# PacificBiosciences/ccs

Measured on AMD Instinct MI355X. Metric: ZMWs/sec (HiFi reads/sec), 10-pass x 10 kb synthetic, higher is better.
Workload: dtype f32

## Files before the change

ccs_amd/csrc/ccsx_api.cpp:

```cpp
#include <hip/hip_runtime.h>

#include <algorithm>
#include <cmath>
#include <cstdio>
#include <cstdlib>
#include <cstring>
#include <initializer_list>
#include <mutex>
#include <string>
#include <vector>

#include "ccsx.h"
#include "ccsx_internal.h"
#include "ccsx_kernels.h"

#define HIPTRY(expr)                                                                                           \
    do {                                                                                                       \
        hipError_t e_ = (expr);                                                                                \
        if (e_ != hipSuccess) {                                                                                \
            ccsx_set_error(std::string(#expr) + ": " + hipGetErrorString(e_));                                 \
            return -2;                                                                                         \
        }                                                                                                      \
    } while (0)

// ... 330 lines not shown
    for (int z = 0; z < b->n_zmw; ++z)
        if (b->read_off[z + 1] < b->read_off[z]) { ccsx_set_error("ccsx_upload: read_off not monotone"); return -1; }
    const int R = b->read_off[b->n_zmw];
    if (R != b->n_reads) { ccsx_set_error("ccsx_upload: n_reads != read_off[n_zmw]"); return -1; }
    for (int r = 0; r < R; ++r)
        if (b->base_off[r + 1] < b->base_off[r]) { ccsx_set_error("ccsx_upload: base_off not monotone"); return -1; }
    if (b->base_off[R] != b->n_bases) { ccsx_set_error("ccsx_upload: n_bases != base_off[n_reads]"); return -1; }
    for (int z = 0; z < b->n_zmw; ++z) {
        bool partial = false;
        for (int r = b->read_off[z]; r < b->read_off[z + 1]; ++r) {
            if (b->flags[r] & 2) partial = true;
            else if (partial) { ccsx_set_error("ccsx_upload: a full-length pass follows a partial pass (flags bit 1) in a ZMW"); return -1; }
        }
    }
    return 0;
}


static int layout(Slot &S, const ccsx_batch *b, int top, BatchTotals *out)
{
    const int n = b->n_zmw, R = b->n_reads;
    if (S.read_zmw.resize(R > 0 ? R : 1) || S.vcap.resize(n) || S.dcap.resize(n) || S.seq_off.assign(n + 1, 0) || S.wb_off.assign(n + 1, 0) ||
        S.ent_off.assign(R + 1, 0) || S.read_off.resize(n + 1) || S.base_off.resize(R + 1) || S.zperm.resize(n) || S.rperm.resize(R > 0 ? R : 1))
        return -2;
    BatchTotals &T = *out;
    T = BatchTotals{};
    ccsx_for_each_zmw_caps(b, [&](int z, const ccsx_zmw_caps &c) {
        S.dcap[z] = (int32_t)c.dcap;
        S.vcap[z] = (int32_t)c.vcap;
        S.seq_off[z + 1] = S.seq_off[z] + S.dcap[z];
        S.wb_off[z + 1] = S.wb_off[z] + (int32_t)c.wcap;
        const int need = 2 * ((int)c.wcap - 1);
        for (int r = b->read_off[z]; r < b->read_off[z + 1]; ++r) {
            S.read_zmw[r] = z;
            S.ent_off[r + 1] = S.ent_off[r] + ((need + 3) & ~3);
        }
        T.nr_max = std::max(T.nr_max, std::min(b->read_off[z + 1] - b->read_off[z], top)); T.need_max = std::max(T.need_max, need);
        T.maxL_max = std::max(T.maxL_max, c.maxL); T.vcap_max = std::max<int64_t>(T.vcap_max, S.vcap[z]); T.dcap_max = std::max<int64_t>(T.dcap_max, S.dcap[z]);
    });
    if (T.maxL_max > 65535) { ccsx_set_error("ccsx_upload: subreads longer than 65535 bases are not supported"); return -1; }
    std::memcpy(S.read_off.p, b->read_off, (size_t)(n + 1) * 4);
    std::memcpy(S.base_off.p, b->base_off, (size_t)(R + 1) * 8);
    T.total_wslots = (int64_t)S.wb_off[n] - n; T.cap_total = S.seq_off[n];
    auto order_by = [](PinVec<int32_t> &perm, size_t cnt_items, auto len_of) {
        const int NBK = 258;
        std::vector<int32_t> cnt(NBK + 1, 0);
        auto cls = [&](int64_t l) { int c = (int)(l >> 8); return NBK - 1 - (c > NBK - 1 ? NBK - 1 : c); };
        for (size_t i = 0; i < cnt_items; ++i) ++cnt[cls(len_of(i)) + 1];
        for (int i = 0; i < NBK; ++i) cnt[i + 1] += cnt[i];
        for (size_t i = 0; i < cnt_items; ++i) perm[cnt[cls(len_of(i))]++] = (int32_t)i;
    };
    order_by(S.zperm, (size_t)n, [&](size_t z) { return (int64_t)S.dcap[z]; });
    if (R > 0) order_by(S.rperm, (size_t)R, [&](size_t r) { return b->base_off[r + 1] - b->base_off[r]; });
    std::vector<int32_t> qpack; std::vector<int64_t> qlen;
    for (int z = 0; z < n; ++z) {
        const int r0 = b->read_off[z];
        int nr = std::min(b->read_off[z + 1] - r0, top);
        while (nr > 0 && (b->flags[r0 + nr - 1] & 2)) --nr;
        for (int g = 0; g < nr; g += 4) {
            const int c = std::min(4, nr - g);
            int64_t ml = 0;
            for (int q = 0; q < c; ++q) ml = std::max<int64_t>(ml, b->base_off[r0 + g + q + 1] - b->base_off[r0 + g + q]);
            qpack.push_back(((r0 + g) << 2) | (c - 1)); qlen.push_back(ml);
        }
    }
    T.n_quads = (int)qpack.size();
    if (S.quads.resize(T.n_quads > 0 ? T.n_quads : 1)) return -2;
    if (T.n_quads > 0) {
        if (S.qperm.resize(T.n_quads)) return -2;
        order_by(S.qperm, (size_t)T.n_quads, [&](size_t q) { return qlen[q]; });
        for (int q = 0; q < T.n_quads; ++q) S.quads[q] = qpack[S.qperm[q]];
    }
    if (T.total_wslots > 0x7fff0000ll) { ccsx_set_error("ccsx_upload: batch too large (more than 2^31 window slots): split it"); return -1; }
    return 0;
}

static int32_t sdust_mask_words(ccsx_handle h, const Slot &S)
{
    const int64_t longest = longest_draft(h, S, 16), words = (longest + 31) / 32;
    if ((int64_t)CCSX_SDUST_TABLE_BYTES + 4 * words <= 160 * 1024) return (int32_t)words;
    ccsx_set_error("tandem-repeat detection: drafts of up to " + std::to_string(longest) + " bases need more LDS than a CU has (lower opts.max_length)");
    return -1;
}

#define RES(dst, buf, bytes) do { if ((buf).reserve(bytes)) return -2; (dst) = (decltype(dst))(buf).p; } while (0)

static int upload_inputs(Slot &S, const ccsx_batch *b, bool kin, hipStream_t st, KParams &P)
{
    const size_t n = (size_t)b->n_zmw, R = (size_t)b->n_reads, R1 = R > 0 ? R : 1, NB = (size_t)b->n_bases;
#define UP(dst, buf, src, bytes) do { RES(dst, buf, bytes); HIPTRY(hipMemcpyAsync((buf).p, (src), (bytes), hipMemcpyHostToDevice, st)); } while (0)
    UP(P.snr, S.d_snr, b->snr, n * 16);
    UP(P.read_off, S.d_read_off, b->read_off, (n + 1) * 4);
    UP(P.base_off, S.d_base_off, b->base_off, (R + 1) * 8);
    UP(P.bases, S.d_bases, b->bases, NB);
    UP(P.pw, S.d_pw, b->pw, NB);
    if (kin) UP(P.ipd, S.d_ipd, b->ipd, NB);
    UP(P.flags, S.d_flags, b->flags, R1);
    UP(P.read_zmw, S.d_read_zmw, S.read_zmw.p, R1 * 4);
    UP(P.vcap, S.d_vcap, S.vcap.p, n * 4);
    UP(P.dcap, S.d_dcap, S.dcap.p, n * 4);
    UP(P.seq_off, S.d_seq_off, S.seq_off.p, (n + 1) * 8);
    UP(P.wb_off, S.d_wb_off, S.wb_off.p, (n + 1) * 4);
    UP(P.ent_off, S.d_ent_off, S.ent_off.p, (R + 1) * 8);
    UP(P.zmw_perm, S.d_zperm, S.zperm.p, S.zperm.size() * 4);
    UP(P.read_perm, S.d_rperm, S.rperm.p, S.rperm.size() * 4);
    UP(P.quads, S.d_quads, S.quads.p, S.quads.size() * 4);
#undef UP
    return 0;
}

static int reserve_state(Slot &S, size_t n, size_t R, bool kin, bool pile, bool tandem, KParams &P)
{
    const size_t R1 = R > 0 ? R : 1, wins = (size_t)S.T.total_wslots + 1, cap = (size_t)S.T.cap_total, ents = (size_t)(S.ent_off[R] + 1);
    RES(P.tabME, S.d_tabME, n * 192 * 4); RES(P.tabINS, S.d_tabINS, n * 192 * 4); RES(P.tabDL, S.d_tabDL, n * 16 * 4); RES(P.tabZ, S.d_tabZ, n * 32 * 4);
    RES(P.draft, S.d_draft, cap);
    if (carve_planes<int32_t>({&P.draft_len, &P.nwin, &P.zstat, &P.nreads_used, &P.np, &P.zref, &P.nfull}, S.d_zmw_i32, n)) return -2;
    RES(P.wbounds, S.d_wbounds, (size_t)S.wb_off[n] * 4);
    RES(P.wslot_zmw, S.d_wslot, wins * 4 + (n + 2) * 4);
    P.wstart = P.wslot_zmw + wins;
    RES(P.ticket_poa, S.d_ticket, 256);
    P.ticket_align = P.ticket_poa + 1; P.debug = P.ticket_poa + 4; P.phase = (unsigned long long *)(P.ticket_poa + 16);
    RES(P.avalid, S.d_avalid, R1); RES(P.ascore, S.d_ascore, R1 * 4);
    RES(P.align_retry, S.d_retry, (R1 + 16) * 4);
    RES(P.ent, S.d_ent, ents * 4); RES(P.dmask, S.d_dmask, ents * 4);
    RES(P.wseq, S.d_wseq, wins * 32); RES(P.wqv, S.d_wqv, wins * 32 * 4);
    RES(P.wsum, S.d_wsum, wins * 4); RES(P.wmeta, S.d_wmeta, wins * 16);
    RES(P.out_seq, S.d_out_seq, cap); RES(P.out_qual, S.d_out_qual, cap); RES(P.out_raw, S.d_out_raw, cap * 4);
    if (carve_planes<int32_t>({&P.out_status, &P.out_len, &P.out_iters, &P.out_nwin, &P.out_fn, &P.out_rn}, S.d_out_i32, n)) return -2;
    if (carve_planes<float>({&P.out_rq, &P.out_ec}, S.d_out_f32, n)) return -2;
    if (kin || pile) { RES(P.wtpl, S.d_wtpl, wins * 32); RES(P.wtmeta, S.d_wtmeta, wins * 4); }
    if (kin) { RES(P.wkin, S.d_wkin, wins * 32 * 4); RES(P.out_kin, S.d_out_kin, cap * 4); P.kin_plane = S.T.cap_total; }
    if (pile) { RES(P.wpile, S.d_wpile, wins * 32 * 4); RES(P.out_pile, S.d_out_pile, cap * 3); P.pile_plane = S.T.cap_total; }
    if (tandem) { RES(P.tflag, S.d_tflag, n * 4); RES(P.tlen, S.d_tlen, n * 4); }
    return 0;
}
#undef RES

struct SlotSizes { size_t poa_bytes, align_i32, align16_i32; };
struct ScratchPlan { int poa_slots, align_slots, align16_slots, align16_regions; };

static SlotSizes scratch_slot_sizes(const BatchTotals &T)
{
    return {(((size_t)T.vcap_max + 64) * CCSX_POA_BYTES_PER_VERTEX + (size_t)T.maxL_max * 4 + 1024 + 255) & ~(size_t)255,
            (size_t)T.need_max * 128 + 4 * (size_t)T.need_max + 64,
            (size_t)4 * (size_t)ccsx_tb_stride((int)T.dcap_max) + 16};
}

static size_t slots_that_fit(size_t room, size_t per_slot, size_t at_least) { return std::max(at_least, room / per_slot); }
static size_t align16_words(int regions, int slots, size_t slot_i32) { return (size_t)regions * slots * slot_i32; }

static ScratchPlan plan_scratch(size_t budget, int n, int R, int n_quads, const SlotSizes &sz, int opt_poa_slots, bool one_region, int max16)
{
    ScratchPlan p;
    p.poa_slots = std::min(opt_poa_slots > 0 ? opt_poa_slots : 16384, n);
    p.poa_slots = (int)std::min<size_t>((size_t)p.poa_slots, slots_that_fit(budget * 3 / 4, sz.poa_bytes, 1));
    p.align_slots = std::min(4096, std::max(R, 2));
    p.align_slots = (int)std::min<size_t>((size_t)p.align_slots, slots_that_fit(budget / 16, sz.align_i32 * 4, 2));
    const size_t fit = slots_that_fit(std::min<size_t>(budget / 8, (size_t)12 << 30), sz.align16_i32 * 4, 1), nq = (size_t)std::max(n_quads, 1);
    auto equal_launches = [nq](size_t at_most) { const size_t launches = (nq + at_most - 1) / at_most; return (int)((nq + launches - 1) / launches); };
    p.align16_regions = 1;
    if (nq <= fit) p.align16_slots = (int)nq;
    else if (one_region) p.align16_slots = equal_launches(fit);
    else { p.align16_slots = equal_launches(std::max<size_t>(1, fit / 2)); p.align16_regions = 2; }
    if (max16 > 0 && p.align16_slots > max16) { p.align16_slots = max16; p.align16_regions = 2; }
    return p;
}

static void bind_scratch(ccsx_handle h, KParams &P)
{
    P.poa_scratch = (uint8_t *)h->d_poa.p; P.align_scratch = (int32_t *)h->d_align.p;
    P.retry_scratch = P.align_scratch + align16_words(P.align16_regions, P.align16_slots, P.align16_slot_i32);
}

static int grow_scratch(ccsx_handle h, int n, int R, const BatchTotals &T, KParams &P)
{
    const SlotSizes sz = scratch_slot_sizes(T);
    static const bool one_region = [] { const char *e = getenv("CCSX_A16_ONE_REGION"); return e && e[0] == '1'; }();
    static const int max16 = [] { const char *e = getenv("CCSX_ALIGN16_MAX_SLOTS"); const int v = e ? atoi(e) : 0; return v > 0 ? v : 0; }();
    std::lock_guard<std::mutex> lk(g_scratch_mutex);
    size_t freeb = 0, totalb = 0;
    HIPTRY(hipMemGetInfo(&freeb, &totalb));
    freeb /= (size_t)h->handles_on_device;
    freeb += h->d_poa.cap + h->d_align.cap;
    ScratchPlan p = plan_scratch(freeb > (size_t)6 << 30 ? freeb - ((size_t)4 << 30) : freeb / 2, n, R, T.n_quads, sz, h->opts.poa_slots, one_region, max16);
    const size_t need_align = ((size_t)p.align_slots * sz.align_i32 + align16_words(p.align16_regions, p.align16_slots, sz.align16_i32)) * 4;
    if ((size_t)p.poa_slots * sz.poa_bytes > h->d_poa.cap || need_align > h->d_align.cap) {
        HIPTRY(hipStreamSynchronize(h->s_draft));
        HIPTRY(hipStreamSynchronize(h->s_comp));
        for (int attempt = 0;; ++attempt) {
            if (h->d_poa.reserve((size_t)p.poa_slots * sz.poa_bytes) == 0) break;
            if (attempt >= 4 || p.poa_slots <= 1) return -2;
            p.poa_slots = std::max(1, p.poa_slots / 2);
        }
        if (h->d_align.reserve(need_align)) return -2;
    }
    P.poa_slot_bytes = sz.poa_bytes; P.poa_slots = p.poa_slots;
    P.align_slot_i32 = sz.align_i32; P.align_slots = p.align_slots;
    P.align16_slot_i32 = sz.align16_i32; P.align16_slots = p.align16_slots; P.align16_regions = p.align16_regions;
// ... 884 lines not shown
```

ccs_amd/csrc/ccsx_internal.h:

```cpp
#pragma once
#include <algorithm>
#include <cstdint>
#include <string>

#include "ccsx.h"

void ccsx_set_error(const std::string &s);

static inline int64_t ccsx_draft_cap(int64_t maxL) { return maxL + maxL / 4 + 64; }
static inline int64_t ccsx_vertex_cap(int64_t maxL) { return (5 * maxL) / 2 + 256; }

struct ccsx_zmw_caps { int64_t maxL, dcap, vcap, wcap; };
static inline ccsx_zmw_caps ccsx_caps_of(int64_t maxL)
{
    const int64_t dcap = ccsx_draft_cap(maxL);
    return {maxL, dcap, ccsx_vertex_cap(maxL), dcap / (CCSX_WIN_CORE - 3) + 4};
}
template <typename F> static inline void ccsx_for_each_zmw_caps(const ccsx_batch *b, F f)
{
    for (int z = 0; z < b->n_zmw; ++z) {
        int64_t maxL = 0;
        for (int r = b->read_off[z]; r < b->read_off[z + 1]; ++r) maxL = std::max<int64_t>(maxL, b->base_off[r + 1] - b->base_off[r]);
        f(z, ccsx_caps_of(maxL));
    }
}
```

ccs_amd/csrc/ccsx_kernels.h:

```cpp
#pragma once
#include <hip/hip_runtime.h>
#include <stdint.h>
#include <math.h>

#include "ccsx.h"

#define CCSX_POA_BYTES_PER_VERTEX 238

static inline float ccsx_perr_floor(int max_qv) { return max_qv == 50 ? 1e-5f : (float)pow(10.0, -(double)max_qv / 10.0); }

#define CCSX_TB_WORDS_PER_BLOCK 18
static inline __host__ __device__ int ccsx_tb_blocks(int Ld) { return (Ld + 15) >> 4; }
static inline __host__ __device__ int ccsx_tb_stride(int Ld) { return (ccsx_tb_blocks(Ld) * CCSX_TB_WORDS_PER_BLOCK + 3) & ~3; }

static inline __host__ __device__ int ccsx_top_passes(int top_passes) { return (top_passes <= 0 || top_passes > CCSX_MAX_PASSES) ? CCSX_MAX_PASSES : top_passes; }

struct KParams {
    int32_t n_zmw, n_reads;
    int32_t maxL_max;
    int32_t vcap_max;
    int32_t need_max;
    int32_t max_reads;
    int32_t qv_only;
    ccsx_opts opts;
    float perr_floor;
    const ccsx_model *model;
    const float *snr;
    const int32_t *read_off;
    const int64_t *base_off;
    const uint8_t *bases, *pw, *flags;
    const int32_t *read_zmw;
    const int32_t *vcap;
    const int32_t *dcap;
    const int64_t *seq_off;
    const int32_t *wb_off;
    const int64_t *ent_off;
    int32_t *wslot_zmw;
    int32_t *wstart;
    float *tabME, *tabINS, *tabDL;
    float *tabZ;
    uint8_t *draft;
    int32_t *draft_len, *nwin, *zstat, *nreads_used, *wbounds, *np;
    int32_t *nfull;
    int32_t *zref;
    int32_t *ticket_poa, *ticket_align;
    int32_t *debug;
    unsigned long long *phase;
    uint8_t *poa_scratch;
    size_t poa_slot_bytes;
    int32_t poa_slots;
    int32_t *align_scratch;
    size_t align_slot_i32;
    int32_t align_slots;
    uint8_t *avalid;
    int32_t *ascore;
    int32_t *ent;
    uint32_t *dmask;
    long long total_wslots;
    int32_t pw_obs_bytes, pw_gb_floats;
    uint8_t *wseq;
    float *wqv;
    float *wsum;
    int4 *wmeta;
    uint8_t *out_seq, *out_qual;
    float *out_raw;
    int32_t *out_status, *out_len, *out_iters, *out_nwin;
// ... 88 lines not shown
```

ccs_amd/csrc/ccsx_kernels.hip:

```cpp
#include <hip/hip_runtime.h>
#include <stdint.h>
#include <cstdio>
#include <cstdlib>

#include "ccsx.h"
#include "ccsx_kernels.h"
#include "wave_ops.h"

#define LANDED(x) asm volatile("" : "+v"(x))

#if (defined(CCSX_EXP_NO_FILL) || defined(CCSX_EXP_NO_SCORE) || defined(CCSX_EXP_ONE_ROUND) || defined(CCSX_EXP_ALL_VALID) || defined(CCSX_EXP_CHEAP_VALIDITY) || \
     defined(CCSX_EXP_NO_ROWS) || defined(CCSX_EXP_NO_SCORE_LOG) || defined(CCSX_EXP_SKIP_ROUND2_SCORE) || defined(CCSX_EXP_NO_QV_EXP) || defined(CCSX_EXP_REPEAT) || defined(CCSX_EXP_NO_BANDMASK) || \
     defined(CCSX_EXP_HOT_PROLOGUE) || defined(CCSX_EXIT_AFTER_PROLOGUE)) && !defined(CCSX_EXPERIMENT)
#error "CCSX_EXP_* / CCSX_EXIT_AFTER_PROLOGUE switches produce wrong results: build them with -DCCSX_EXPERIMENT (never ship such a library)"
#endif
#define CCSX_STR2(x) #x
#define CCSX_STR(x) CCSX_STR2(x)
int ccsx_kernel_is_experiment()
{
#ifdef CCSX_EXPERIMENT
    return 1;
#else
    return 0;
#endif
// ... 1177 lines not shown
            unsigned insbits = bitj | (bitj << 1);
            if (need) {
                OMsave[(size_t)kk * 64 + lane] = make_int2(org, (int)kd);
                if (lane == 0) lo_need[kk] = lo;
                org = i;
                kd = 0u; insbits = 0x80000001u; ecol = j;
            }
            const int d0 = best + 4 * lane;
            const int dc = d0 > -(1 << 24) ? d0 : -(1 << 24);
            const int key = wave_scan_max_i32((dc << 6) | lane);
            const int xi = (key >> 6) - 4 * lane;
            const int ksl = key & 63;
            const int osrc = __shfl(org, ksl);
            const unsigned ksrc = (unsigned)__shfl((int)kd, ksl);
            if (xi > best) { best = xi; org = osrc; kd = ksrc | insbits; }
            if (i > I || best < -(1 << 22)) best = NEGV;
            const int cm = wave_reduce_max_i32(best);
            const unsigned long long bal = __ballot(best == cm);
            br = lo + (__ffsll((long long)bal) - 1);
            Mprev = best; Oprev = org; Kprev = kd;
            if (need) {
                const int ebest = rl(org, br - lo);
                if (lane == 0) { cm_need[kk] = cm; br_need[kk] = br; eb_need[kk] = ebest; }
                ++kk;
                next_need = (kk >= nneed) ? -1 : rfl(need_at(kk));
            }
        };
        { int jj = 0; for (; jj + 2 <= nblk; jj += 2) { column(jj); column(jj + 1); } if (jj < nblk) column(jj); }
    }
    AlignEnd out; out.M = Mprev; out.O = Oprev; out.K = Kprev; out.lo = lo;
    return out;
}

#define AB16 16
#define NEG16 (-(1 << 23))
#define AB16_ABOVE 6
#define AB16_SAT_ROWS 1
#define AB16_SAT_GAIN 1
#define AVALID_TB 2
__device__ __forceinline__ int tb_blocks(int Ld) { return ccsx_tb_blocks(Ld); }
__device__ __forceinline__ int tb_stride(int Ld) { return ccsx_tb_stride(Ld); }
__device__ __forceinline__ unsigned shift_in(unsigned acc, unsigned long long m)
{
    unsigned r; unsigned long long co;
    asm("v_addc_co_u32_e64 %0, %1, %2, %2, %3" : "=v"(r), "=s"(co) : "v"(acc), "s"(m));
    return r;
}
__device__ __forceinline__ int sel_i32(unsigned long long m, int a, int b)
{
    int r;
    asm("v_cndmask_b32_e64 %0, %1, %2, %3" : "=v"(r) : "v"(b), "v"(a), "s"(m));
    return r;
}
__global__ __launch_bounds__(64) void k_align16(KParams P, int qbase, int pass, int region)
{
    const int lane = threadIdx.x, h = lane >> 4, l = lane & 15, rowb = lane & 48;
    uint32_t *sread = dyn_lds;
    uint32_t *Osave = (uint32_t *)(P.align_scratch + ((size_t)region * P.align16_slots + blockIdx.x) * P.align16_slot_i32);
    if (qbase + (int)blockIdx.x >= P.n_quads) return;
    const int qd = rfl(P.quads[qbase + blockIdx.x]);
    const int rfirst = qd >> 2, nq = (qd & 3) + 1;
    const int z = rfl(P.read_zmw[rfirst]);
    const int r0 = rfl(P.read_off[z]);
    const int zr = rfl(P.zref[z]);
    if (pass && !(zr & ZREF_PASSBIT(pass))) return;
    const bool live = h < nq;
    const int r = rfirst + (live ? h : 0);
    if (live && l == 0) { P.avalid[r] = 0; P.ascore[r] = NEGV; }
    if (P.zstat[z] != CCSX_SUCCESS) return;
    const int nused = rfl(P.nreads_used[z]);
    if (rfirst - r0 >= nused) return;
    const bool use = live && (r - r0 < nused);
    if (P.opts.disable_heuristics || (P.tflag && (rfl(P.tflag[z]) & 2))) {
        if (l == 0 && use) { const int idx = atomicAdd(&P.align_retry[0], 1); P.align_retry[16 + idx] = r; }
        return;
    }
    const int Ld = rfl(P.draft_len[z]), nw = rfl(P.nwin[z]);
    const uint8_t *d = P.draft + P.seq_off[z];
    const int32_t *wb = P.wbounds + P.wb_off[z];
    const int wstride = CH16 / 16 + 3;
    const int fl0 = rfl(P.flags[r0 + (zr & 255)] & 1);
    for (int hh = 0; hh < nq; ++hh) {
        const int rr = rfirst + hh;
        const int Ih = rfl((int)(P.base_off[rr + 1] - P.base_off[rr]));
        load_read_chunk(sread + hh * wstride + 1, P.bases + P.base_off[rr], Ih, rfl(((P.flags[rr] & 1) != fl0) ? 1 : 0), 0, lane);
    }
    if (lane < 4) sread[lane * wstride] = 0u;
    __syncthreads();
    int c0 = 0;
    int bi = l - 1;
    const int I = use ? (int)(P.base_off[r + 1] - P.base_off[r]) : 0;
    const uint32_t *myread = sread + h * wstride + 1;
    const int nneed = 2 * nw;
    const int tbs = tb_stride(Ld);
    uint32_t *mvL = Osave + (size_t)h * tbs + l;
    uint32_t *shL = Osave + (size_t)h * tbs + tb_blocks(Ld) * 16;
    unsigned mvacc = 0u, shacc = 0u, edgeacc = 0u;
    bool prev_edge = false;
    int kk = 1;
    int kkb = 1;
    int needv = need_col(wb, nw, Ld, (kkb + lane < nneed) ? kkb + lane : nneed - 1);
    int next_need = rl(needv, 0);
    int Mprev = (l <= I) ? l * SC_INS : NEG16;
    int lo = 0, br = 0;
    const int hiI = I - (AB16 - 1) > 0 ? I - (AB16 - 1) : 0;
    const int lane4 = 4 * lane;
    const bool tiny = __any(use && I < AB16 - 1);
    int satf = 0, cmE0 = 0, cmE1 = 0;
    unsigned long long satm = 0ull;
    for (int jb = 0; jb < Ld; jb += LANES) {
        const int dL = (jb + lane < Ld) ? d[jb + lane] : 0;
        asm volatile("" :: "v"(dL));
        const unsigned long long dB0 = __ballot(dL & 1), dB1 = __ballot(dL & 2);
        const int nblk = (Ld - jb) < LANES ? (Ld - jb) : LANES;
        auto column = [&](const int jj) {
            const int j = jb + jj + 1;
            const int plo = lo;
            {
                int t = br + 1 - AB16_ABOVE;
                t = t > plo ? t : plo;
                t = t < plo + 2 ? t : plo + 2;
                lo = t < hiI ? t : hiI;
            }
            const int sh = lo - plo;
            bi += sh;
            shacc = (shacc << 2) | (unsigned)sh;
            edgeacc = (edgeacc << 2) | (prev_edge ? 1u : 0u);
            prev_edge = j == next_need;
            const int vb = (int)((dB0 >> jj) & 1ull) | ((int)((dB1 >> jj) & 1ull) << 1);
            if ((jj & 7) == 0 && __any(lo + AB16 + 2 + 16 > c0 + CH16)) {
                for (int hh = 0; hh < nq; ++hh) {
                    const int src = hh << 4;
                    if (rl(lo, src) + AB16 + 2 + 16 > rl(c0, src) + CH16) {
                        const int rr = rfirst + hh;
                        const int Ih = rfl((int)(P.base_off[rr + 1] - P.base_off[rr]));
                        const int nc0 = rl(lo, src) - 16 > 0 ? rl(lo, src) - 16 : 0;
                        __syncthreads();
                        load_read_chunk(sread + hh * wstride + 1, P.bases + P.base_off[rr], Ih, rfl(((P.flags[rr] & 1) != fl0) ? 1 : 0), nc0, lane);
                        __syncthreads();
                        if (h == hh) { c0 = nc0; bi = lo + l - 1 - nc0; }
                    }
                }
            }
            const uint32_t bw = myread[bi >> 4];
            const int rbv = (int)((bw >> (2 * (bi & 15))) & 3u);
            const unsigned long long matchm = __builtin_amdgcn_uicmp((unsigned)vb, (unsigned)rbv, 32 );
            int x, y;
            if (__all(sh == 1)) {
                x = Mprev; y = row_shl1_i32(Mprev, NEG16);
            } else {
                const int mR = row_shr1_i32(Mprev, NEG16), m1 = row_shl1_i32(Mprev, NEG16);
                const bool s0 = sh == 0, s1 = sh == 1;
                x = s0 ? mR : (s1 ? Mprev : m1);
                const int yu = row_shl1_i32(x, NEG16);
                y = s0 ? Mprev : yu;
            }
            const int dg = x + sel_i32(matchm, SC_MATCH, SC_MISMATCH);
            const int dl = y + SC_DEL;
            const unsigned long long delm = __builtin_amdgcn_sicmp(dl, dg, 38 );
            int best = dl > dg ? dl : dg;
            const int xi = row_scan_max_i32(best + lane4) - lane4;
            const unsigned long long insm = __builtin_amdgcn_sicmp(xi, best, 38 );
            best = xi > best ? xi : best;
            mvacc = shift_in(mvacc, delm | insm);
            mvacc = shift_in(mvacc, insm | ~(delm | matchm));
            if ((jj & 15) == 15) {
                *mvL = mvacc; mvL += 16;
                if (l == 0) *(uint2 *)shL = make_uint2(shacc, edgeacc);
                shL += 2;
            }
            if (tiny && lo + l > I) best = NEG16;
            const int ck = row_allmax_i32((best << 4) | (15 - l));
            const int cm = ck >> 4, brl = 15 - (ck & 15);
            br = lo + brl;
            satm |= __builtin_amdgcn_sicmp(brl, AB16 - AB16_SAT_ROWS, 39 ) & __builtin_amdgcn_sicmp(lo, hiI, 40 );
            Mprev = best;
            if (j == next_need) {
                if (kk >= 2 && cm - cmE0 < AB16_SAT_GAIN) satf = 1;
                cmE0 = cmE1; cmE1 = cm;
                ++kk;
                if (kk - kkb >= LANES) { kkb = kk; needv = need_col(wb, nw, Ld, (kkb + lane < nneed) ? kkb + lane : nneed - 1); }
                next_need = (kk >= nneed) ? -1 : rl(needv, kk - kkb);
            }
        };
        { int jj = 0; for (; jj + 2 <= nblk; jj += 2) { column(jj); column(jj + 1); } if (jj < nblk) column(jj); }
    }
    if (Ld & 15) {
        const int s2 = 2 * (16 - (Ld & 15));
        *mvL = mvacc << s2;
        if (l == 0) *(uint2 *)shL = make_uint2(shacc << s2, edgeacc << s2);
    }
    const int oe = I - lo;
    const bool inr = oe >= 0 && oe < AB16;
    const int srcl = rowb + (inr ? oe : 0);
    const int scv = __shfl(Mprev, srcl);
    satf |= (int)((satm >> lane) & 1ull);
    const int sc = (inr && scv > -(1 << 22)) ? scv : NEGV;
    const int valid = (sc > NEGV / 2 && sc >= Ld && !satf) ? 1 : 0;
    if (l == 0 && use) {
        P.ascore[r] = sc;
        if (valid) {
            Osave[4 * (size_t)tbs + h] = (uint32_t)lo;
            P.avalid[r] = AVALID_TB;
        } else {
            P.avalid[r] = 0;
            const int idx = atomicAdd(&P.align_retry[0], 1);
            P.align_retry[16 + idx] = r;
        }
    }
}

#define TBE 2
#define TB_LSTRIDE (TBE * 16 + 2 * TBE + 1)
__global__ __launch_bounds__(64) void k_align16_tb(KParams P, int qbase, int nslots, int region)
{
    __shared__ uint32_t sS[64 * TB_LSTRIDE];
    __shared__ unsigned long long sOff[64];
    __shared__ int sCnt[64];
    const int lane = threadIdx.x;
    const int t = (int)blockIdx.x * 64 + lane;
    const int s = t >> 2, h = t & 3;
    bool act = s < nslots;
    int r = 0;
    if (act) {
        const int qd = P.quads[qbase + s];
        const int rfirst = qd >> 2, nq = (qd & 3) + 1;
        act = h < nq;
        r = rfirst + (act ? h : 0);
        act = act && P.avalid[r] == AVALID_TB;
    }
    if (!__any(act)) return;
    const int z = act ? P.read_zmw[r] : 0;
    const int Ld = act ? P.draft_len[z] : 0, nw = act ? P.nwin[z] : 1;
    const int I = act ? (int)(P.base_off[r + 1] - P.base_off[r]) : 0;
    const int tbs = tb_stride(Ld), nb = tb_blocks(Ld);
    const size_t sbase = ((size_t)region * P.align16_slots + s) * P.align16_slot_i32;
    const size_t moff = sbase + (size_t)h * tbs;
    const uint32_t *As = (const uint32_t *)P.align_scratch;
    const uint32_t *shw = As + moff + (size_t)nb * 16;
    int lo = act ? (int)As[sbase + 4 * (size_t)tbs + h] : 0;
    int32_t *ent = P.ent + P.ent_off[r];
    uint32_t *dm = P.dmask + P.ent_off[r];
    const int nneed = 2 * nw;
    uint32_t *my = sS + lane * TB_LSTRIDE;
    uint32_t *mySh = my + TBE * 16;
    uint32_t e0 = 0u, e1 = 0u, e2r = 0u, e3 = 0u, d0 = 0u, d1 = 0u, d2 = 0u, d3 = 0u;
    int i = I, j = act ? Ld : 0, K = nneed - 1;
    int eH = Ld;
    unsigned mk = 0u, pend = 0u;
    bool atedge = true;
    int bhi = nb;
    while (__any(j > 0)) {
        const bool on = j > 0;
        const int b0 = bhi > 0 ? (bhi - 1) & ~1 : 0;
        sOff[lane] = on ? (unsigned long long)(moff + (size_t)b0 * 16) : 0ull;
        sCnt[lane] = on ? (bhi - b0) * 16 : 0;
        const uint4 vs = *(const uint4 *)(on ? shw + 2 * b0 : As);
        __syncthreads();
        uint4 vm[TBE * 4];
#pragma unroll
        for (int q = 0; q < TBE * 4; ++q) {
            const int rd = q * (16 / TBE) + lane / (TBE * 4), part = lane % (TBE * 4);
            vm[q] = *(const uint4 *)(As + sOff[rd] + (part * 4 < sCnt[rd] ? part * 4 : 0));
        }
        mySh[0] = vs.x; mySh[1] = vs.y; mySh[2] = vs.z; mySh[3] = vs.w;
#pragma unroll
        for (int q = 0; q < TBE * 4; ++q) {
            const int rd = q * (16 / TBE) + lane / (TBE * 4), part = lane % (TBE * 4);
            if (part * 4 < sCnt[rd]) {
                uint32_t *dst = sS + rd * TB_LSTRIDE + part * 4;
                dst[0] = vm[q].x; dst[1] = vm[q].y; dst[2] = vm[q].z; dst[3] = vm[q].w;
            }
        }
        __syncthreads();
        const int jstop = b0 * 16;
        while (j > jstop) {
            const int blk = ((j - 1) >> 4) - b0, o = (i - lo) & 15;
            int sft = 2 * (15 - ((j - 1) & 15));
            const uint32_t Wm = my[blk * 16 + o], Ws = mySh[2 * blk], We = mySh[2 * blk + 1];
            if (!atedge) {
                uint32_t bad = (Wm >> sft) | ((Ws >> sft) ^ 0x55555555u) | ((We >> sft) & 0x55555555u);
                bad = (bad | (bad >> 1)) & 0x55555555u;
                const int k = bad ? (__ffs((int)bad) - 1) >> 1 : 16;
                if (k > 0) {
                    i -= k; j -= k; lo -= k; sft += 2 * k;
                    if (i < 0) { j = 0; continue; }
                    if (sft >= 32) continue;
                }
            }
            const int code = (int)(Wm >> sft) & 3;
            const unsigned w2 = Ws >> sft, e2 = We >> sft;
            const bool ins = code == 3;
            const unsigned bj = 1u << ((eH - j) & 31);
// ... 2591 lines not shown
```

ccs_amd/csrc/wave_ops.h:

```cpp
#pragma once
#include <hip/hip_runtime.h>

#define DPP_ROW_SHR(n) (0x110 + (n))
#define DPP_WAVE_SHL1 0x130
#define DPP_WAVE_SHR1 0x138
#define DPP_ROW_BCAST15 0x142
#define DPP_ROW_BCAST31 0x143

__device__ __forceinline__ int wave_shr1_i32(int x, int fill) { return __builtin_amdgcn_update_dpp(fill, x, DPP_WAVE_SHR1, 0xf, 0xf, false); }
__device__ __forceinline__ int wave_shl1_i32(int x, int fill) { return __builtin_amdgcn_update_dpp(fill, x, DPP_WAVE_SHL1, 0xf, 0xf, false); }
__device__ __forceinline__ float wave_shr1_f32(float x, float fill) { return __int_as_float(wave_shr1_i32(__float_as_int(x), __float_as_int(fill))); }
__device__ __forceinline__ float wave_shl1_f32(float x, float fill) { return __int_as_float(wave_shl1_i32(__float_as_int(x), __float_as_int(fill))); }

__device__ __forceinline__ float wave_shr1_f32_z(float x) { return __int_as_float(__builtin_amdgcn_mov_dpp(__float_as_int(x), DPP_WAVE_SHR1, 0xf, 0xf, true)); }
__device__ __forceinline__ float wave_shl1_f32_z(float x) { return __int_as_float(__builtin_amdgcn_mov_dpp(__float_as_int(x), DPP_WAVE_SHL1, 0xf, 0xf, true)); }

#define DPP_ROW_ROR(n) (0x120 + (n))
__device__ __forceinline__ float row_ror1_f32(float x) { return __int_as_float(__builtin_amdgcn_mov_dpp(__float_as_int(x), DPP_ROW_ROR(1), 0xf, 0xf, false)); }
__device__ __forceinline__ float row_rol1_f32(float x) { return __int_as_float(__builtin_amdgcn_mov_dpp(__float_as_int(x), DPP_ROW_ROR(15), 0xf, 0xf, false)); }

__device__ __forceinline__ int wave_shr1_i32_z(int x) { return __builtin_amdgcn_mov_dpp(x, DPP_WAVE_SHR1, 0xf, 0xf, true); }
__device__ __forceinline__ int wave_shl1_i32_z(int x) { return __builtin_amdgcn_mov_dpp(x, DPP_WAVE_SHL1, 0xf, 0xf, true); }

__device__ __forceinline__ int imax(int a, int b) { return a > b ? a : b; }
// ... 2 lines not shown
__device__ __forceinline__ int wave_scan_max_i32(int v)
{
    int s = imax(v, __builtin_amdgcn_update_dpp(WAVE_IMIN, v, DPP_ROW_SHR(1), 0xf, 0xf, false));
    s = imax(s, __builtin_amdgcn_update_dpp(WAVE_IMIN, s, DPP_ROW_SHR(2), 0xf, 0xf, false));
    s = imax(s, __builtin_amdgcn_update_dpp(WAVE_IMIN, s, DPP_ROW_SHR(4), 0xf, 0xf, false));
    s = imax(s, __builtin_amdgcn_update_dpp(WAVE_IMIN, s, DPP_ROW_SHR(8), 0xf, 0xf, false));
    s = imax(s, __builtin_amdgcn_update_dpp(WAVE_IMIN, s, DPP_ROW_BCAST15, 0xa, 0xf, false));
    s = imax(s, __builtin_amdgcn_update_dpp(WAVE_IMIN, s, DPP_ROW_BCAST31, 0xc, 0xf, false));
    return s;
}
__device__ __forceinline__ int half_scan_max_i32(int v)
{
    int s = imax(v, __builtin_amdgcn_update_dpp(WAVE_IMIN, v, DPP_ROW_SHR(1), 0xf, 0xf, false));
    s = imax(s, __builtin_amdgcn_update_dpp(WAVE_IMIN, s, DPP_ROW_SHR(2), 0xf, 0xf, false));
    s = imax(s, __builtin_amdgcn_update_dpp(WAVE_IMIN, s, DPP_ROW_SHR(4), 0xf, 0xf, false));
    s = imax(s, __builtin_amdgcn_update_dpp(WAVE_IMIN, s, DPP_ROW_SHR(8), 0xf, 0xf, false));
    s = imax(s, __builtin_amdgcn_update_dpp(WAVE_IMIN, s, DPP_ROW_BCAST15, 0xa, 0xf, false));
    return s;
}
__device__ __forceinline__ int wave_scan_add_i32(int v)
{
    int s = v + __builtin_amdgcn_update_dpp(0, v, DPP_ROW_SHR(1), 0xf, 0xf, false);
    s = s + __builtin_amdgcn_update_dpp(0, v, DPP_ROW_SHR(2), 0xf, 0xf, false);
    s = s + __builtin_amdgcn_update_dpp(0, v, DPP_ROW_SHR(3), 0xf, 0xf, false);
    s = s + __builtin_amdgcn_update_dpp(0, s, DPP_ROW_SHR(4), 0xf, 0xe, false);
    s = s + __builtin_amdgcn_update_dpp(0, s, DPP_ROW_SHR(8), 0xf, 0xc, false);
    s = s + __builtin_amdgcn_update_dpp(0, s, DPP_ROW_BCAST15, 0xa, 0xf, false);
    s = s + __builtin_amdgcn_update_dpp(0, s, DPP_ROW_BCAST31, 0xc, 0xf, false);
    return s;
}
#define DPP_ROW_SHL(n) (0x100 + (n))
__device__ __forceinline__ int row_shr1_i32(int x, int fill) { return __builtin_amdgcn_update_dpp(fill, x, DPP_ROW_SHR(1), 0xf, 0xf, false); }
__device__ __forceinline__ int row_shl1_i32(int x, int fill) { return __builtin_amdgcn_update_dpp(fill, x, DPP_ROW_SHL(1), 0xf, 0xf, false); }
__device__ __forceinline__ int row_shl2_i32(int x, int fill) { return __builtin_amdgcn_update_dpp(fill, x, DPP_ROW_SHL(2), 0xf, 0xf, false); }
__device__ __forceinline__ int row_shr1_i32_z(int x) { return __builtin_amdgcn_mov_dpp(x, DPP_ROW_SHR(1), 0xf, 0xf, true); }
__device__ __forceinline__ int row_shl1_i32_z(int x) { return __builtin_amdgcn_mov_dpp(x, DPP_ROW_SHL(1), 0xf, 0xf, true); }
__device__ __forceinline__ int row_shl2_i32_z(int x) { return __builtin_amdgcn_mov_dpp(x, DPP_ROW_SHL(2), 0xf, 0xf, true); }
__device__ __forceinline__ int row_scan_max_i32(int v)
{
    int s = imax(v, __builtin_amdgcn_update_dpp(WAVE_IMIN, v, DPP_ROW_SHR(1), 0xf, 0xf, false));
    s = imax(s, __builtin_amdgcn_update_dpp(WAVE_IMIN, s, DPP_ROW_SHR(2), 0xf, 0xf, false));
    s = imax(s, __builtin_amdgcn_update_dpp(WAVE_IMIN, s, DPP_ROW_SHR(4), 0xf, 0xf, false));
    s = imax(s, __builtin_amdgcn_update_dpp(WAVE_IMIN, s, DPP_ROW_SHR(8), 0xf, 0xf, false));
    return s;
}
__device__ __forceinline__ int row_allmax_i32(int v)
{
    int s = imax(v, __builtin_amdgcn_update_dpp(WAVE_IMIN, v, DPP_ROW_ROR(1), 0xf, 0xf, false));
    s = imax(s, __builtin_amdgcn_update_dpp(WAVE_IMIN, s, DPP_ROW_ROR(2), 0xf, 0xf, false));
    s = imax(s, __builtin_amdgcn_update_dpp(WAVE_IMIN, s, DPP_ROW_ROR(4), 0xf, 0xf, false));
    s = imax(s, __builtin_amdgcn_update_dpp(WAVE_IMIN, s, DPP_ROW_ROR(8), 0xf, 0xf, false));
    return s;
}

__device__ __forceinline__ int wave_reduce_max_i32(int v) { return __builtin_amdgcn_readlane(wave_scan_max_i32(v), 63); }
__device__ __forceinline__ int wave_reduce_add_i32(int v) { return __builtin_amdgcn_readlane(wave_scan_add_i32(v), 63); }

#define WAVE_PAIR_STEP(SRC_D, SRC_O, CTRL, RM, BM)                                                    \
    {                                                                                                 \
        const int td = __builtin_amdgcn_update_dpp(d, SRC_D, CTRL, RM, BM, false);                    \
        const int to = __builtin_amdgcn_update_dpp(o, SRC_O, CTRL, RM, BM, false);                    \
        const bool take = td > d;                                                                     \
        d = take ? td : d; o = take ? to : o;                                                         \
    }
__device__ __forceinline__ void wave_scan_max_pair(int &d, int &o)
{
    const int d0 = d, o0 = o;
    WAVE_PAIR_STEP(d0, o0, DPP_ROW_SHR(1), 0xf, 0xf)
    WAVE_PAIR_STEP(d0, o0, DPP_ROW_SHR(2), 0xf, 0xf)
    WAVE_PAIR_STEP(d0, o0, DPP_ROW_SHR(3), 0xf, 0xf)
    WAVE_PAIR_STEP(d, o, DPP_ROW_SHR(4), 0xf, 0xe)
    WAVE_PAIR_STEP(d, o, DPP_ROW_SHR(8), 0xf, 0xc)
    WAVE_PAIR_STEP(d, o, DPP_ROW_BCAST15, 0xa, 0xf)
    WAVE_PAIR_STEP(d, o, DPP_ROW_BCAST31, 0xc, 0xf)
}
```

Baseline: 38470.

## Pack leftover reads from different ZMWs into mixed align16 quads

Quads used to hold up to four consecutive reads of one ZMW, so ZMWs whose pass count was not a multiple of four left partly empty 64-lane waves. Full groups of four now stay per-ZMW, and the leftover reads of all ZMWs are packed together into shared quads stored as four explicit read indices. A templated mixed-ZMW path handles per-row drafts, window bounds and lengths, and the kernel gains a waves-per-EU attribute. The mixed path carries per-row draft broadcast and bookkeeping overhead, and quad storage grows fourfold.

```diff
diff --git a/ccs_amd/csrc/ccsx_api.cpp b/ccs_amd/csrc/ccsx_api.cpp
--- a/ccs_amd/csrc/ccsx_api.cpp
+++ b/ccs_amd/csrc/ccsx_api.cpp
@@ -406,24 +406,14 @@
     };
     order_by(S.zperm, (size_t)n, [&](size_t z) { return (int64_t)S.dcap[z]; });
     if (R > 0) order_by(S.rperm, (size_t)R, [&](size_t r) { return b->base_off[r + 1] - b->base_off[r]; });
-    std::vector<int32_t> qpack; std::vector<int64_t> qlen;
-    for (int z = 0; z < n; ++z) {
-        const int r0 = b->read_off[z];
-        int nr = std::min(b->read_off[z + 1] - r0, top);
-        while (nr > 0 && (b->flags[r0 + nr - 1] & 2)) --nr;
-        for (int g = 0; g < nr; g += 4) {
-            const int c = std::min(4, nr - g);
-            int64_t ml = 0;
-            for (int q = 0; q < c; ++q) ml = std::max<int64_t>(ml, b->base_off[r0 + g + q + 1] - b->base_off[r0 + g + q]);
-            qpack.push_back(((r0 + g) << 2) | (c - 1)); qlen.push_back(ml);
-        }
-    }
-    T.n_quads = (int)qpack.size();
-    if (S.quads.resize(T.n_quads > 0 ? T.n_quads : 1)) return -2;
+    std::vector<int32_t> qrows; std::vector<int64_t> qlen;
+    ccsx_pack_quads(n, b->read_off, b->base_off, b->flags, top, qrows, qlen);
+    T.n_quads = (int)qlen.size();
+    if (S.quads.resize(T.n_quads > 0 ? 4 * (size_t)T.n_quads : 4)) return -2;
     if (T.n_quads > 0) {
         if (S.qperm.resize(T.n_quads)) return -2;
         order_by(S.qperm, (size_t)T.n_quads, [&](size_t q) { return qlen[q]; });
-        for (int q = 0; q < T.n_quads; ++q) S.quads[q] = qpack[S.qperm[q]];
+        for (int q = 0; q < T.n_quads; ++q) std::memcpy(S.quads.p + 4 * (size_t)q, qrows.data() + 4 * (size_t)S.qperm[q], 16);
     }
     if (T.total_wslots > 0x7fff0000ll) { ccsx_set_error("ccsx_upload: batch too large (more than 2^31 window slots): split it"); return -1; }
     return 0;
@@ -497,7 +487,7 @@
 {
     return {(((size_t)T.vcap_max + 64) * CCSX_POA_BYTES_PER_VERTEX + (size_t)T.maxL_max * 4 + 1024 + 255) & ~(size_t)255,
             (size_t)T.need_max * 128 + 4 * (size_t)T.need_max + 64,
-            (size_t)4 * (size_t)ccsx_tb_stride((int)T.dcap_max) + 16};
+            ccsx_a16_slot_words((int)T.dcap_max)};
 }
 
 static size_t slots_that_fit(size_t room, size_t per_slot, size_t at_least) { return std::max(at_least, room / per_slot); }
diff --git a/ccs_amd/csrc/ccsx_internal.h b/ccs_amd/csrc/ccsx_internal.h
--- a/ccs_amd/csrc/ccsx_internal.h
+++ b/ccs_amd/csrc/ccsx_internal.h
@@ -2,6 +2,7 @@
 #include <algorithm>
 #include <cstdint>
 #include <string>
+#include <vector>
 
 #include "ccsx.h"
 
@@ -24,3 +25,25 @@
         f(z, ccsx_caps_of(maxL));
     }
 }
+
+static inline void ccsx_pack_quads(int n_zmw, const int32_t *read_off, const int64_t *base_off, const uint8_t *flags, int top, std::vector<int32_t> &rows,
+                                   std::vector<int64_t> &len)
+{
+    rows.clear(); len.clear();
+    auto used = [&](int z) {
+        int nr = std::min(read_off[z + 1] - read_off[z], top);
+        while (nr > 0 && (flags[read_off[z] + nr - 1] & 2)) --nr;
+        return nr;
+    };
+    auto put = [&](int r, int row) {
+        if (row == 0) { rows.insert(rows.end(), 4, -1); len.push_back(0); }
+        rows[rows.size() - 4 + row] = r;
+        len.back() = std::max<int64_t>(len.back(), base_off[r + 1] - base_off[r]);
+    };
+    for (int z = 0; z < n_zmw; ++z)
+        for (int g = 0, nr = used(z); g + 4 <= nr; g += 4)
+            for (int q = 0; q < 4; ++q) put(read_off[z] + g + q, q);
+    int row = 0;
+    for (int z = 0; z < n_zmw; ++z)
+        for (int nr = used(z), g = nr & ~3; g < nr; ++g, row = (row + 1) & 3) put(read_off[z] + g, row);
+}
diff --git a/ccs_amd/csrc/ccsx_kernels.h b/ccs_amd/csrc/ccsx_kernels.h
--- a/ccs_amd/csrc/ccsx_kernels.h
+++ b/ccs_amd/csrc/ccsx_kernels.h
@@ -12,6 +12,8 @@
 #define CCSX_TB_WORDS_PER_BLOCK 18
 static inline __host__ __device__ int ccsx_tb_blocks(int Ld) { return (Ld + 15) >> 4; }
 static inline __host__ __device__ int ccsx_tb_stride(int Ld) { return (ccsx_tb_blocks(Ld) * CCSX_TB_WORDS_PER_BLOCK + 3) & ~3; }
+static inline __host__ __device__ size_t ccsx_a16_slot_words(int dcap_max) { return (size_t)4 * (size_t)ccsx_tb_stride(dcap_max) + 16; }
+static inline __host__ __device__ int ccsx_a16_row_stride(size_t slot_words) { return (int)((slot_words - 16) >> 2); }
 
 static inline __host__ __device__ int ccsx_top_passes(int top_passes) { return (top_passes <= 0 || top_passes > CCSX_MAX_PASSES) ? CCSX_MAX_PASSES : top_passes; }
 
diff --git a/ccs_amd/csrc/ccsx_kernels.hip b/ccs_amd/csrc/ccsx_kernels.hip
--- a/ccs_amd/csrc/ccsx_kernels.hip
+++ b/ccs_amd/csrc/ccsx_kernels.hip
@@ -1253,69 +1253,128 @@
     asm("v_cndmask_b32_e64 %0, %1, %2, %3" : "=v"(r) : "v"(b), "v"(a), "s"(m));
     return r;
 }
-__global__ __launch_bounds__(64) void k_align16(KParams P, int qbase, int pass, int region)
+template <bool MX>
+__device__ __forceinline__ void align16_wave(const KParams &P, const int pass, uint32_t *const Osave, const int rp0, const int rp1, const int rp2, const int rp3)
 {
     const int lane = threadIdx.x, h = lane >> 4, l = lane & 15, rowb = lane & 48;
     uint32_t *sread = dyn_lds;
-    uint32_t *Osave = (uint32_t *)(P.align_scratch + ((size_t)region * P.align16_slots + blockIdx.x) * P.align16_slot_i32);
-    if (qbase + (int)blockIdx.x >= P.n_quads) return;
-    const int qd = rfl(P.quads[qbase + blockIdx.x]);
-    const int rfirst = qd >> 2, nq = (qd & 3) + 1;
-    const int z = rfl(P.read_zmw[rfirst]);
-    const int r0 = rfl(P.read_off[z]);
-    const int zr = rfl(P.zref[z]);
-    if (pass && !(zr & ZREF_PASSBIT(pass))) return;
-    const bool live = h < nq;
-    const int r = rfirst + (live ? h : 0);
-    if (live && l == 0) { P.avalid[r] = 0; P.ascore[r] = NEGV; }
-    if (P.zstat[z] != CCSX_SUCCESS) return;
-    const int nused = rfl(P.nreads_used[z]);
-    if (rfirst - r0 >= nused) return;
-    const bool use = live && (r - r0 < nused);
-    if (P.opts.disable_heuristics || (P.tflag && (rfl(P.tflag[z]) & 2))) {
-        if (l == 0 && use) { const int idx = atomicAdd(&P.align_retry[0], 1); P.align_retry[16 + idx] = r; }
-        return;
-    }
-    const int Ld = rfl(P.draft_len[z]), nw = rfl(P.nwin[z]);
-    const uint8_t *d = P.draft + P.seq_off[z];
-    const int32_t *wb = P.wbounds + P.wb_off[z];
+    const int rst = ccsx_a16_row_stride(P.align16_slot_i32);
     const int wstride = CH16 / 16 + 3;
-    const int fl0 = rfl(P.flags[r0 + (zr & 255)] & 1);
-    for (int hh = 0; hh < nq; ++hh) {
-        const int rr = rfirst + hh;
+    int r, Ld, nw, Lmax, nq = 4, fl0 = 0;
+    bool use;
+    const uint8_t *d;
+    const int32_t *wb = P.wbounds;
+    int wbo = 0;
+    if constexpr (!MX) {
+        const int rfirst = rp0;
+        nq = 1 + (rp1 >= 0 ? 1 : 0) + (rp2 >= 0 ? 1 : 0) + (rp3 >= 0 ? 1 : 0);
+        const int z = rfl(P.read_zmw[rfirst]);
+        const int r0 = rfl(P.read_off[z]);
+        const int zr = rfl(P.zref[z]);
+        if (pass && !(zr & ZREF_PASSBIT(pass))) return;
+        const bool live = h < nq;
+        r = rfirst + (live ? h : 0);
+        if (live && l == 0) { P.avalid[r] = 0; P.ascore[r] = NEGV; }
+        if (P.zstat[z] != CCSX_SUCCESS) return;
+        const int nused = rfl(P.nreads_used[z]);
+        if (rfirst - r0 >= nused) return;
+        use = live && (r - r0 < nused);
+        if (P.opts.disable_heuristics || (P.tflag && (rfl(P.tflag[z]) & 2))) {
+            if (l == 0 && use) { const int idx = atomicAdd(&P.align_retry[0], 1); P.align_retry[16 + idx] = r; }
+            return;
+        }
+        Ld = rfl(P.draft_len[z]); nw = rfl(P.nwin[z]);
+        d = P.draft + P.seq_off[z];
+        wb = P.wbounds + P.wb_off[z];
+        fl0 = rfl(P.flags[r0 + (zr & 255)] & 1);
+        Lmax = Ld;
+    } else {
+        const int rq = h == 0 ? rp0 : (h == 1 ? rp1 : (h == 2 ? rp2 : rp3));
+        const bool live = rq >= 0;
+        r = live ? rq : rp0;
+        const int z = P.read_zmw[r];
+        const int zr = P.zref[z];
+        const bool mine = live && !(pass && !(zr & ZREF_PASSBIT(pass)));
+        if (mine && l == 0) { P.avalid[r] = 0; P.ascore[r] = NEGV; }
+        use = mine && P.zstat[z] == CCSX_SUCCESS && (r - P.read_off[z] < P.nreads_used[z]);
+        if (P.opts.disable_heuristics || P.tflag) {
+            const bool wide = use && (P.opts.disable_heuristics || (P.tflag[z] & 2));
+            if (wide && l == 0) { const int idx = atomicAdd(&P.align_retry[0], 1); P.align_retry[16 + idx] = r; }
+            use = use && !wide;
+        }
+        if (!__any(use)) return;
+        Ld = use ? P.draft_len[z] : 0;
+        nw = P.nwin[z];
+        d = P.draft + P.seq_off[z];
+        wbo = P.wb_off[z];
+        const int a = rl(Ld, 0), b = rl(Ld, 16), c = rl(Ld, 32), e = rl(Ld, 48);
+        const int ab = a > b ? a : b, ce = c > e ? c : e;
+        Lmax = ab > ce ? ab : ce;
+    }
+    auto load_row = [&](const int hh, const int nc0) {
+        int rr, f0;
+        if constexpr (!MX) { rr = rp0 + hh; f0 = fl0; }
+        else {
+            rr = hh == 0 ? rp0 : (hh == 1 ? rp1 : (hh == 2 ? rp2 : rp3));
+            const int zz = rfl(P.read_zmw[rr]);
+            f0 = rfl(P.flags[rfl(P.read_off[zz]) + (rfl(P.zref[zz]) & 255)] & 1);
+        }
         const int Ih = rfl((int)(P.base_off[rr + 1] - P.base_off[rr]));
-        load_read_chunk(sread + hh * wstride + 1, P.bases + P.base_off[rr], Ih, rfl(((P.flags[rr] & 1) != fl0) ? 1 : 0), 0, lane);
-    }
+        load_read_chunk(sread + hh * wstride + 1, P.bases + P.base_off[rr], Ih, rfl(((P.flags[rr] & 1) != f0) ? 1 : 0), nc0, lane);
+    };
+    auto row_runs = [&](const int hh) { if constexpr (MX) return rl(Ld, hh << 4) > 0; else return true; };
+    for (int hh = 0; hh < nq; ++hh) if (row_runs(hh)) load_row(hh, 0);
     if (lane < 4) sread[lane * wstride] = 0u;
     __syncthreads();
-    int c0 = 0;
+    int c0 = MX ? 1 - l : 0;
     int bi = l - 1;
     const int I = use ? (int)(P.base_off[r + 1] - P.base_off[r]) : 0;
     const uint32_t *myread = sread + h * wstride + 1;
     const int nneed = 2 * nw;
-    const int tbs = tb_stride(Ld);
-    uint32_t *mvL = Osave + (size_t)h * tbs + l;
-    uint32_t *shL = Osave + (size_t)h * tbs + tb_blocks(Ld) * 16;
+    uint32_t *mvL = Osave + (size_t)h * rst + l;
+    uint32_t *shL = Osave + (size_t)h * rst + tb_blocks(Ld) * 16;
+    const int moff = h * rst + l;
+    auto soff = [&]() { return moff - l + tb_blocks(Ld) * 16; };
+    auto need_row = [&](const int k) { return need_col(wb + wbo, nneed >> 1, Ld, k < nneed ? k : nneed - 1); };
     unsigned mvacc = 0u, shacc = 0u, edgeacc = 0u;
     bool prev_edge = false;
+    unsigned pedge = 0u;
     int kk = 1;
-    int kkb = 1;
-    int needv = need_col(wb, nw, Ld, (kkb + lane < nneed) ? kkb + lane : nneed - 1);
-    int next_need = rl(needv, 0);
+    int kkb = 1, needv = 0, next_need, nn1 = 0;
+    if constexpr (!MX) {
+        needv = need_col(wb, nw, Ld, (kkb + lane < nneed) ? kkb + lane : nneed - 1);
+        next_need = rl(needv, 0);
+    } else {
+        next_need = use ? need_row(1) : -1;
+        if (use) nn1 = need_row(2);
+    }
     int Mprev = (l <= I) ? l * SC_INS : NEG16;
+    int Mfin = Mprev;
     int lo = 0, br = 0;
-    const int hiI = I - (AB16 - 1) > 0 ? I - (AB16 - 1) : 0;
+    int hiI = I - (AB16 - 1) > 0 ? I - (AB16 - 1) : 0;
     const int lane4 = 4 * lane;
     const bool tiny = __any(use && I < AB16 - 1);
     int satf = 0, cmE0 = 0, cmE1 = 0;
     unsigned long long satm = 0ull;
-    for (int jb = 0; jb < Ld; jb += LANES) {
-        const int dL = (jb + lane < Ld) ? d[jb + lane] : 0;
-        asm volatile("" :: "v"(dL));
-        const unsigned long long dB0 = __ballot(dL & 1), dB1 = __ballot(dL & 2);
-        const int nblk = (Ld - jb) < LANES ? (Ld - jb) : LANES;
+    unsigned dw = 0u, dnx = 0u;
+    if constexpr (MX) dnx = (l < Ld) ? (unsigned)(d[l] & 3) : 0u;
+    for (int jb = 0; jb < Lmax; jb += LANES) {
+        unsigned long long dB0 = 0ull, dB1 = 0ull;
+        if constexpr (!MX) {
+            const int dL = (jb + lane < Ld) ? d[jb + lane] : 0;
+            asm volatile("" :: "v"(dL));
+            dB0 = __ballot(dL & 1); dB1 = __ballot(dL & 2);
+        }
+        const int nblk = (Lmax - jb) < LANES ? (Lmax - jb) : LANES;
         auto column = [&](const int jj) {
             const int j = jb + jj + 1;
+            if constexpr (MX) {
+                if ((jj & 15) == 0) {
+                    dw = (unsigned)row_allor_i32((int)(dnx << (2 * l)));
+                    const int jn = jb + jj + 16 + l;
+                    dnx = (jn < Ld) ? (unsigned)(d[jn] & 3) : 0u;
+                }
+            }
             const int plo = lo;
             {
                 int t = br + 1 - AB16_ABOVE;
@@ -1324,22 +1383,28 @@
                 lo = t < hiI ? t : hiI;
             }
             const int sh = lo - plo;
+            if constexpr (MX) bi = lo - c0; else
             bi += sh;
             shacc = (shacc << 2) | (unsigned)sh;
-            edgeacc = (edgeacc << 2) | (prev_edge ? 1u : 0u);
-            prev_edge = j == next_need;
-            const int vb = (int)((dB0 >> jj) & 1ull) | ((int)((dB1 >> jj) & 1ull) << 1);
-            if ((jj & 7) == 0 && __any(lo + AB16 + 2 + 16 > c0 + CH16)) {
+            int vb;
+            if constexpr (!MX) {
+                edgeacc = (edgeacc << 2) | (prev_edge ? 1u : 0u);
+                prev_edge = j == next_need;
+                vb = (int)((dB0 >> jj) & 1ull) | ((int)((dB1 >> jj) & 1ull) << 1);
+            } else {
+                edgeacc = (edgeacc << 2) | pedge;
+                pedge = (j == next_need) ? 1u : 0u;
+                vb = (int)((dw >> (2 * (jj & 15))) & 3u);
+            }
+            if ((jj & 7) == 0 && __any(lo + AB16 + 2 + 16 > c0 + (MX ? l - 1 : 0) + CH16)) {
                 for (int hh = 0; hh < nq; ++hh) {
                     const int src = hh << 4;
-                    if (rl(lo, src) + AB16 + 2 + 16 > rl(c0, src) + CH16) {
-                        const int rr = rfirst + hh;
-                        const int Ih = rfl((int)(P.base_off[rr + 1] - P.base_off[rr]));
+                    if (row_runs(hh) && rl(lo, src) + AB16 + 2 + 16 > rl(c0, src) - (MX ? 1 : 0) + CH16) {
                         const int nc0 = rl(lo, src) - 16 > 0 ? rl(lo, src) - 16 : 0;
                         __syncthreads();
-                        load_read_chunk(sread + hh * wstride + 1, P.bases + P.base_off[rr], Ih, rfl(((P.flags[rr] & 1) != fl0) ? 1 : 0), nc0, lane);
+                        load_row(hh, nc0);
                         __syncthreads();
-                        if (h == hh) { c0 = nc0; bi = lo + l - 1 - nc0; }
+                        if (h == hh) { c0 = MX ? nc0 - (l - 1) : nc0; bi = lo + l - 1 - nc0; }
                     }
                 }
             }
@@ -1366,9 +1431,15 @@
             mvacc = shift_in(mvacc, delm | insm);
             mvacc = shift_in(mvacc, insm | ~(delm | matchm));
             if ((jj & 15) == 15) {
-                *mvL = mvacc; mvL += 16;
-                if (l == 0) *(uint2 *)shL = make_uint2(shacc, edgeacc);
-                shL += 2;
+                if constexpr (!MX) {
+                    *mvL = mvacc; mvL += 16;
+                    if (l == 0) *(uint2 *)shL = make_uint2(shacc, edgeacc);
+                    shL += 2;
+                } else if (j <= Ld) {
+                    const int blk = (jb + jj) >> 4;
+                    Osave[moff + 16 * blk] = mvacc;
+                    if (l == 0) *(uint2 *)(Osave + soff() + 2 * blk) = make_uint2(shacc, edgeacc);
+                }
             }
             if (tiny && lo + l > I) best = NEG16;
             const int ck = row_allmax_i32((best << 4) | (15 - l));
@@ -1376,32 +1447,54 @@
             br = lo + brl;
             satm |= __builtin_amdgcn_sicmp(brl, AB16 - AB16_SAT_ROWS, 39 ) & __builtin_amdgcn_sicmp(lo, hiI, 40 );
             Mprev = best;
-            if (j == next_need) {
-                if (kk >= 2 && cm - cmE0 < AB16_SAT_GAIN) satf = 1;
-                cmE0 = cmE1; cmE1 = cm;
-                ++kk;
-                if (kk - kkb >= LANES) { kkb = kk; needv = need_col(wb, nw, Ld, (kkb + lane < nneed) ? kkb + lane : nneed - 1); }
-                next_need = (kk >= nneed) ? -1 : rl(needv, kk - kkb);
+            if constexpr (!MX) {
+                if (j == next_need) {
+                    if (kk >= 2 && cm - cmE0 < AB16_SAT_GAIN) satf = 1;
+                    cmE0 = cmE1; cmE1 = cm;
+                    ++kk;
+                    if (kk - kkb >= LANES) { kkb = kk; needv = need_col(wb, nw, Ld, (kkb + lane < nneed) ? kkb + lane : nneed - 1); }
+                    next_need = (kk >= nneed) ? -1 : rl(needv, kk - kkb);
+                }
+            } else {
+                if (j == next_need) {
+                    satm |= __ballot(kk >= 2 && cm - cmE0 < AB16_SAT_GAIN);
+                    cmE0 = cmE1; cmE1 = cm;
+                    ++kk;
+                    next_need = (kk >= nneed) ? -1 : nn1;
+                    nn1 = need_row(kk + 1);
+                }
+                if (j == Ld) {
+                    if (Ld & 15) {
+                        const int s2 = 2 * (16 - (Ld & 15)), blk = (jb + jj) >> 4;
+                        Osave[moff + 16 * blk] = mvacc << s2;
+                        if (l == 0) *(uint2 *)(Osave + soff() + 2 * blk) = make_uint2(shacc << s2, edgeacc << s2);
+                    }
+                    Mfin = best; hiI = lo;
+                }
             }
         };
         { int jj = 0; for (; jj + 2 <= nblk; jj += 2) { column(jj); column(jj + 1); } if (jj < nblk) column(jj); }
     }
-    if (Ld & 15) {
-        const int s2 = 2 * (16 - (Ld & 15));
-        *mvL = mvacc << s2;
-        if (l == 0) *(uint2 *)shL = make_uint2(shacc << s2, edgeacc << s2);
+    if constexpr (!MX) {
+        if (Ld & 15) {
+            const int s2 = 2 * (16 - (Ld & 15));
+            *mvL = mvacc << s2;
+            if (l == 0) *(uint2 *)shL = make_uint2(shacc << s2, edgeacc << s2);
+        }
+        Mfin = Mprev;
     }
     const int oe = I - lo;
     const bool inr = oe >= 0 && oe < AB16;
     const int srcl = rowb + (inr ? oe : 0);
-    const int scv = __shfl(Mprev, srcl);
+    const int scv = __shfl(Mfin, srcl);
     satf |= (int)((satm >> lane) & 1ull);
     const int sc = (inr && scv > -(1 << 22)) ? scv : NEGV;
     const int valid = (sc > NEGV / 2 && sc >= Ld && !satf) ? 1 : 0;
+    if constexpr (MX) r = h == 0 ? rp0 : (h == 1 ? rp1 : (h == 2 ? rp2 : rp3));
     if (l == 0 && use) {
         P.ascore[r] = sc;
         if (valid) {
-            Osave[4 * (size_t)tbs + h] = (uint32_t)lo;
+            Osave[4 * (size_t)rst + h] = (uint32_t)lo;
             P.avalid[r] = AVALID_TB;
         } else {
             P.avalid[r] = 0;
@@ -1409,6 +1502,18 @@
             P.align_retry[16 + idx] = r;
         }
     }
+}
+
+__global__ __launch_bounds__(64) __attribute__((amdgpu_waves_per_eu(8, 8))) void k_align16(KParams P, int qbase, int pass, int region)
+{
+    uint32_t *Osave = (uint32_t *)(P.align_scratch + ((size_t)region * P.align16_slots + blockIdx.x) * P.align16_slot_i32);
+    if (qbase + (int)blockIdx.x >= P.n_quads) return;
+    const int4 q = ((const int4 *)P.quads)[qbase + blockIdx.x];
+    const int rp0 = rfl(q.x), rp1 = rfl(q.y), rp2 = rfl(q.z), rp3 = rfl(q.w);
+    const int z0 = rfl(P.read_zmw[rp0]);
+    const bool mixed = (rp1 >= 0 && rfl(P.read_zmw[rp1]) != z0) || (rp2 >= 0 && rfl(P.read_zmw[rp2]) != z0) || (rp3 >= 0 && rfl(P.read_zmw[rp3]) != z0);
+    if (mixed) align16_wave<true>(P, pass, Osave, rp0, rp1, rp2, rp3);
+    else align16_wave<false>(P, pass, Osave, rp0, rp1, rp2, rp3);
 }
 
 #define TBE 2
@@ -1424,22 +1529,22 @@
     bool act = s < nslots;
     int r = 0;
     if (act) {
-        const int qd = P.quads[qbase + s];
-        const int rfirst = qd >> 2, nq = (qd & 3) + 1;
-        act = h < nq;
-        r = rfirst + (act ? h : 0);
+        const int rq = P.quads[4 * (size_t)(qbase + s) + h];
+        act = rq >= 0;
+        r = act ? rq : 0;
         act = act && P.avalid[r] == AVALID_TB;
     }
     if (!__any(act)) return;
     const int z = act ? P.read_zmw[r] : 0;
     const int Ld = act ? P.draft_len[z] : 0, nw = act ? P.nwin[z] : 1;
     const int I = act ? (int)(P.base_off[r + 1] - P.base_off[r]) : 0;
-    const int tbs = tb_stride(Ld), nb = tb_blocks(Ld);
+    const int nb = tb_blocks(Ld);
+    const int rst = ccsx_a16_row_stride(P.align16_slot_i32);
     const size_t sbase = ((size_t)region * P.align16_slots + s) * P.align16_slot_i32;
-    const size_t moff = sbase + (size_t)h * tbs;
+    const size_t moff = sbase + (size_t)h * rst;
     const uint32_t *As = (const uint32_t *)P.align_scratch;
     const uint32_t *shw = As + moff + (size_t)nb * 16;
-    int lo = act ? (int)As[sbase + 4 * (size_t)tbs + h] : 0;
+    int lo = act ? (int)As[sbase + 4 * (size_t)rst + h] : 0;
     int32_t *ent = P.ent + P.ent_off[r];
     uint32_t *dm = P.dmask + P.ent_off[r];
     const int nneed = 2 * nw;
diff --git a/ccs_amd/csrc/wave_ops.h b/ccs_amd/csrc/wave_ops.h
--- a/ccs_amd/csrc/wave_ops.h
+++ b/ccs_amd/csrc/wave_ops.h
@@ -78,6 +78,14 @@
     s = imax(s, __builtin_amdgcn_update_dpp(WAVE_IMIN, s, DPP_ROW_ROR(8), 0xf, 0xf, false));
     return s;
 }
+__device__ __forceinline__ int row_allor_i32(int v)
+{
+    int s = v | __builtin_amdgcn_update_dpp(0, v, DPP_ROW_ROR(1), 0xf, 0xf, false);
+    s = s | __builtin_amdgcn_update_dpp(0, s, DPP_ROW_ROR(2), 0xf, 0xf, false);
+    s = s | __builtin_amdgcn_update_dpp(0, s, DPP_ROW_ROR(4), 0xf, 0xf, false);
+    s = s | __builtin_amdgcn_update_dpp(0, s, DPP_ROW_ROR(8), 0xf, 0xf, false);
+    return s;
+}
 
 __device__ __forceinline__ int wave_reduce_max_i32(int v) { return __builtin_amdgcn_readlane(wave_scan_max_i32(v), 63); }
 __device__ __forceinline__ int wave_reduce_add_i32(int v) { return __builtin_amdgcn_readlane(wave_scan_add_i32(v), 63); }
```

After: 38890, median of 6. +1.1%, better.
